# jdapena/distributed_point_functions

Measured on AMD Instinct MI355X. Metric: DPF leaf evals/sec, full-domain 2^30 uint64 at 1/2/4/8 GPUs; AES blocks/s, higher is better.
Workload: dtype u64

## Files before the change

distributed_point_functions_amd/csrc/kernels/dpf_device.h:

```cpp
#pragma once
#include <hip/hip_runtime.h>
#include <stdint.h>
#include <string.h>

#include "../../../include/dpf_hip.h"
#include "aes_core.h"

namespace {

struct T0Table {
  uint32_t v[256];
};
constexpr T0Table make_t0() {
  T0Table t{};
  for (int i = 0; i < 256; ++i) {
    uint32_t s = dpf_aes::kSbox[i];
    uint32_t s2 = ((s << 1) ^ ((s & 0x80) ? 0x1b : 0)) & 0xff;
    t.v[i] = s2 | (s << 8) | (s << 16) | ((s2 ^ s) << 24);
  }
  return t;
}
__constant__ T0Table c_t0 = make_t0();

struct RoundKeys {
// ... 136 lines not shown

struct ExpandParams {
  int64_t num_items;
  int num_levels;
  int k0;
  int S;
  const dpf_block* seeds_in;
  const uint8_t* ctrl_in;
  const dpf_block* cw_seed;
  const uint8_t* cw_left;
  const uint8_t* cw_right;
  char* out;
  RoundKeys rkl, rkr, rkv, rkd;
  int dyn_chunks;
  int ph_end[3];
  int64_t ph_item[3];
  unsigned int* chunk_counter;
  unsigned long long* clock;
};

__device__ __forceinline__ int64_t take_expand_chunk(const ExpandParams& p, int* lds_counter,
                                                     int64_t done, int& k0, int& S) {
  unsigned int c = 0;
  if ((threadIdx.x & 63) == 0)
    c = p.chunk_counter ? __hip_atomic_fetch_add(p.chunk_counter, 1u, __ATOMIC_RELAXED,
                                                 __HIP_MEMORY_SCOPE_AGENT)
                        : (unsigned int)atomicAdd(lds_counter, 1);
  c = __builtin_amdgcn_readfirstlane(c);
  const unsigned int e0 = (unsigned int)p.ph_end[0], e1 = (unsigned int)p.ph_end[1],
                     e2 = (unsigned int)p.ph_end[2];
  if (c >= e2) return done;
  const int j = (c >= e0) + (c >= e1);
  const unsigned int first = j == 0 ? 0u : (j == 1 ? e0 : e1);
  const unsigned int last = j == 0 ? e0 : (j == 1 ? e1 : e2);
  const int64_t item0 = j == 0 ? p.ph_item[0] : (j == 1 ? p.ph_item[1] : p.ph_item[2]);
  const int64_t group = p.chunk_counter ? 0 : (int64_t)blockIdx.x;
  const int64_t chunk = group * (int64_t)(last - first) + (c - first);
  k0 = p.k0 + 2 * j;
  S = p.S - 2 * j;
  return item0 + chunk * 64 + (int64_t)(threadIdx.x & 63);
}

__device__ __forceinline__ int64_t take_chunk(int* counter, int64_t per_wg, int64_t chunks,
                                              int64_t done) {
  int c = 0;
  if ((threadIdx.x & 63) == 0) c = atomicAdd(counter, 1);
  c = __builtin_amdgcn_readfirstlane(c);
  const int64_t g = (int64_t)blockIdx.x * per_wg + c;
  return c < per_wg && g < chunks ? g * 64 + (int64_t)(threadIdx.x & 63) : done;
}
// ... 901 lines not shown
```

distributed_point_functions_amd/csrc/kernels/dpf_expand_plan.hip:

```cpp
#include <stdint.h>

#include "../../../include/dpf_hip.h"
#include "dpf_runtime.h"

namespace dpf_rt {

int choose_subtree_depth(int64_t num_starts, int num_levels) {
  const int S = num_levels < max_subtree_depth() ? num_levels : max_subtree_depth();
#if defined(DPF_FORCE_S)
  if (num_levels >= DPF_FORCE_S) return DPF_FORCE_S;
#endif
  double best = -1;
  int best_s = S;
  for (int cand = S; cand >= (num_levels > 0 ? 1 : 0); --cand) {
    const int64_t items = num_starts << (num_levels - cand);
    const int blk = block_for(items);
    const int64_t threads = (int64_t)grid_for(items, blk) * blk;
    const int64_t rounds = (items + threads - 1) / threads;
    const double cost = (double)rounds * (2.0 * (num_levels - cand) + 3.0 * (double)(1ll << cand));
    if (best < 0 || cost < best * 0.999) {
      best = cost;
      best_s = cand;
    }
  }
// ... 2 lines not shown

bool small_shape(int64_t num_starts, int num_levels, int* t, int* D) {
  const int64_t cus = num_cus();
  if (hook_is("DPF_EXPAND_SMALL", '0') || num_levels < 1 || num_starts < 1 || num_starts > cus)
    return false;
  int tt = 0;
  while (tt < num_levels - 1 && (num_starts << (tt + 1)) <= cus) ++tt;
  const int d = num_levels - tt;
  if (d < 1 || d > kSmallMaxD) return false;
  *t = tt;
  *D = d;
  return true;
}

bool top_shape(int64_t num_items, int k0, int* t, int* D) {
  const int64_t starts = num_items >> k0;
  if (hook_is("DPF_EXPAND_TOP", '0') || k0 < 8 || starts > num_cus() ||
      num_items < 4 * (int64_t)num_cus())
    return false;
  int tt = 0;
  while ((starts << tt) < num_cus() && tt < k0 - 1) ++tt;
  if (k0 - tt > kSmallMaxD) tt = k0 - kSmallMaxD;
  if (k0 - tt < 1 || (starts << tt) > INT32_MAX) return false;
  *t = tt;
  *D = k0 - tt;
  return true;
}

static int octet_dynamic_shift(int S) {
  return hook_int("DPF_OCTET_DYNAMIC", S >= 11 ? 4 : 2, 0, 4);
}
int octet_walk_levels() { return hook_int("DPF_OCTET_WALK", 2, 0, 4); }
ChunkPlan plan_chunks(int64_t num_items, int k0, int S, int min_S, int64_t cus, bool sched_ok) {
  ChunkPlan c{};
  const int sh = octet_dynamic_shift(S);
  if (sh <= 0 || S - sh < min_S || k0 + sh > 62 || cus <= 0 || num_items <= 0 ||
      num_items > (INT64_MAX >> (sh + 4)) || (num_items << sh) % (cus * 64) != 0 ||
      (num_items << sh) < 4 * cus * max_block() || (num_items << sh) / 64 > (INT32_MAX >> 4))
    return c;
  c.shift = sh;
  const int big = sched_ok && (num_items << S) / cus >= ((int64_t)1 << 20);
  c.global = hook_int("DPF_OCTET_GLOBAL", big, 0, 1);
  c.groups = c.global ? 1 : cus;
  const int k = k0 + sh, s = S - sh;
  const int64_t coarse = (num_items << sh) / 64;
  const int finer = hook_int("DPF_OCTET_TAPER", big ? 2 : 0, 0, 2);
  const int64_t at = hook_int("DPF_OCTET_TAPER_AT", 2, 1, 16) * cus * (max_block() / 64);
  auto exists = [&](int j) { return j <= finer && s - 2 * j >= min_S && k + 2 * j <= 62; };
  int64_t start[4] = {0, coarse, coarse, coarse};
  if (exists(1)) start[1] = coarse - (coarse < at ? coarse : at);
  if (exists(2)) start[2] = coarse - (coarse - start[1] < (at >> 2) ? coarse - start[1] : (at >> 2));
  for (int j = 0; j < 3; ++j) {
    c.k0[j] = k + 2 * j;
    c.S[j] = s - 2 * j;
    c.chunks[j] = (start[j + 1] - start[j]) << (2 * j);
    c.first_item[j] = (start[j] * 64) << (2 * j);
  }
  return c;
}

void write_plan(const ChunkPlan& c, int64_t* out) {
  for (int i = 0; i < 15; ++i) out[i] = 0;
  out[0] = c.shift;
  if (!c.shift) return;
  out[1] = c.global;
  out[2] = c.groups;
  for (int j = 0; j < 3; ++j) {
    out[3 + 4 * j] = c.chunks[j];
    out[4 + 4 * j] = c.first_item[j];
    out[5 + 4 * j] = c.k0[j];
    out[6 + 4 * j] = c.S[j];
  }
}

}

using namespace dpf_rt;

extern "C" int dpf_hip_octet_schedule(int64_t num_items, int k0, int subtree_depth, int min_depth,
                                      int compute_units, int64_t* out) {
  if (!out) return fail(kInvalidArgument, "NULL pointer");
  if (num_items < 1 || k0 < 0 || subtree_depth < 0 || k0 + subtree_depth > 62 ||
      compute_units < 1)
    return fail(kInvalidArgument, "launch shape out of range");
  write_plan(plan_chunks(num_items, k0, subtree_depth, min_depth, compute_units, true), out);
  return kOk;
}
```

distributed_point_functions_amd/csrc/kernels/dpf_kernels.hip:

```cpp
#include <hip/hip_runtime.h>
#include <stdint.h>
#include <stdlib.h>
#include <string.h>

#include <atomic>
#include <type_traits>
#include <vector>
#include <string>

#include "../../../include/dpf_hip.h"
#include "dpf_device.h"
#include "dpf_dot.h"
#include "dpf_runtime.h"

namespace dpf_rt {
thread_local std::string g_last_error;
thread_local const char* g_last_expand = "";
thread_local int g_last_expand_s = -1;
thread_local int64_t g_last_dynamic_chunks = 0;
std::atomic<unsigned long long*> g_clock_acc{nullptr};

int fail(int code, const std::string& msg) {
  g_last_error = msg;
  return code;
// ... 58 lines not shown
      uint32_t bit = path_bit(path, p.num_levels - 1 - j);
      path_step(lk, lk.ks.l, lk.ks.d, s, t, bit, lds.cw_seed[j], lds.cw_ctrl[j]);
    }
    store_block(p.seeds_out + i, s);
    p.ctrl_out[i] = (uint8_t)t;
  }
}

template <class Leaf, bool SCHED = false>
__global__ __launch_bounds__(kBlock) DPF_WAVES_ATTR void expand_kernel(ExpandParams p, Leaf leaf) {
  __shared__ LdsImage lds;
  __shared__ int next_chunk;
  leaf.init();
  fill_tables(lds.tab);
  fill_cws(lds, p.cw_seed, p.cw_left, p.cw_right, p.num_levels);
  if (threadIdx.x == 0) next_chunk = 0;
  __syncthreads();
  const LdsLookup lk = make_lookup(lds, KeySet{key_ref(p.rkl), key_ref(p.rkr), key_ref(p.rkv), key_ref(p.rkd)});
  int k0 = p.k0, S = p.S;
  if constexpr (SCHED) ClockStamp::first_begin(p.clock);
  const int64_t nch = (p.num_items + 63) / 64;
  const int64_t end = SCHED ? INT64_MAX : p.num_items;
  auto take = [&]() -> int64_t {
    if constexpr (SCHED) return take_expand_chunk(p, &next_chunk, end, k0, S);
    else return take_chunk(&next_chunk, p.dyn_chunks, nch, p.num_items);
  };
  for (int64_t item = SCHED || p.dyn_chunks ? take()
                                            : blockIdx.x * (int64_t)blockDim.x + threadIdx.x;
       item < end;
       item = SCHED || p.dyn_chunks ? take() : item + (int64_t)gridDim.x * blockDim.x) {
    const int B = S >= 1 ? 1 : 0;
    const int G = S - B;
    const int64_t ngroups = (int64_t)1 << G;
    const int64_t r = item >> k0;
    Block4 s = load_block(p.seeds_in + r);
    uint32_t t = p.ctrl_in[r] & 1u;
    for (int j = 0; j < k0; ++j) {
      uint32_t bit = (uint32_t)((item >> (k0 - 1 - j)) & 1);
      path_step(lk, lk.ks.l, lk.ks.d, s, t, bit, lds.cw_seed[j], lds.cw_ctrl[j]);
    }
    Block4 sib[kGMax];
    uint32_t tb = 0;
    const int64_t leaf_base = item << S;
    for (int64_t g = 0; g < ngroups; ++g) {
      Block4 node = s;
      uint32_t nt = t;
      int ds = 0;
      if (g != 0) {
        ds = G - (int)__builtin_ctzll((unsigned long long)g);
#pragma unroll
        for (int d = 1; d <= kGMax; ++d)
          if (d == ds) { node = sib[d - 1]; nt = (tb >> d) & 1u; }
// ... 77 lines not shown
template <> struct OctetStash<SwarLeaf> { static constexpr int value = 1; };

template <class Leaf, bool SCHED = false>
__global__ __launch_bounds__(kBlock) DPF_WAVES_ATTR void expand_octet_kernel(ExpandParams p,
                                                                             Leaf leaf) {
  __shared__ LdsImage lds;
  constexpr int kStash = OctetStash<Leaf>::value;
  __shared__ uint4 stash[kBlock];
  __shared__ uint3 stash2[kStash >= 2 ? kBlock : 1];
  __shared__ int next_chunk;
  static_assert(sizeof(LdsImage) + 16 * kBlock + (kStash >= 2 ? 12 * kBlock : 0) + 16 <= 160 * 1024,
                "LDS over 160 KiB");
  leaf.init();
  fill_tables(lds.tab);
  fill_cws(lds, p.cw_seed, p.cw_left, p.cw_right, p.num_levels);
  if (threadIdx.x == 0) next_chunk = 0;
  __syncthreads();
  const LdsLookup lk = make_lookup(lds, KeySet{key_ref(p.rkl), key_ref(p.rkr), key_ref(p.rkv), key_ref(p.rkd)});
  int k0 = p.k0, S = p.S;
  ClockStamp stamp;
  stamp.begin(p.clock);
  const int lane = (int)(threadIdx.x & 63);
  const int64_t end = SCHED ? INT64_MAX : p.num_items;
  auto take = [&]() -> int64_t {
    if constexpr (SCHED) {
      return take_expand_chunk(p, &next_chunk, end, k0, S);
    } else {
      int c = 0;
      if (lane == 0) c = atomicAdd(&next_chunk, 1);
      c = __builtin_amdgcn_readfirstlane(c);
      return c < p.dyn_chunks ? ((int64_t)blockIdx.x * p.dyn_chunks + c) * 64 + lane
                              : p.num_items;
    }
  };
  for (int64_t item = SCHED || p.dyn_chunks ? take()
                                            : blockIdx.x * (int64_t)blockDim.x + threadIdx.x;
       item < end;
       item = SCHED || p.dyn_chunks ? take() : item + (int64_t)gridDim.x * blockDim.x) {
    const int G = S - 3;
    const int64_t ngroups = (int64_t)1 << G;
    const int64_t r = item >> k0;
    Block4 s = load_block(p.seeds_in + r);
    uint32_t t = p.ctrl_in[r] & 1u;
    for (int j = 0; j < k0; ++j) {
      const uint32_t bit = (uint32_t)((item >> (k0 - 1 - j)) & 1);
      path_step(lk, lk.ks.l, lk.ks.d, s, t, bit, lds.cw_seed[j], lds.cw_ctrl[j]);
    }
    Block4 sib[kGMax];
    uint32_t tb = 0;
    const int64_t leaf_base = item << S;
    Block4 next = s;
    for (int64_t g = 0; g < ngroups; ++g) {
      Block4 node = next;
      uint32_t nt = t;
      int ds = 0;
      if (g != 0) {
        ds = G - (int)__builtin_ctzll((unsigned long long)g);
        nt = (tb >> ds) & 1u;
      }
// ... 36 lines not shown
            q[2] = sib[kGMax - 2];
          }
          const uint4 v = stash[threadIdx.x];
          q[3] = Block4{v.x, v.y, v.z, v.w};
        }
        children_step_x2(lk, lk.ks.l, lk.ks.r, q[2 * hf], qt[2 * hf], q[2 * hf + 1],
                         qt[2 * hf + 1], lds.cw_seed[lvl + 2], lds.cw_ctrl[lvl + 2], l, lt);
        octet_half(leaf, lk, lk.ks.v, l, lt, leaf_base + 8 * g + 4 * hf, p.out, &sib[kGMax - 2]);
      }
    }
  }
  stamp.end(p.clock);
  if constexpr (HasFinish<Leaf>::value) leaf.finish();
}

template <class Leaf> struct IsFastInt : std::false_type {};
template <int BITS, bool XOR> struct IsFastInt<FastIntLeaf<BITS, XOR>> : std::true_type {};
template <int BITS, bool XOR> struct IsFastInt<DotLeaf<BITS, XOR>> : std::true_type {};
template <class Leaf>
__global__ __launch_bounds__(kBlock) DPF_WAVES_ATTR void expand_small_kernel(ExpandParams p, Leaf leaf) {
  __shared__ LdsImage lds;
  __shared__ uint4 nodes[kBlock];
  __shared__ uint32_t tbits[kBlock];
  leaf.init();
  fill_tables(lds.tab);
  fill_cws(lds, p.cw_seed, p.cw_left, p.cw_right, p.num_levels);
  __syncthreads();
  const LdsLookup lk =
      make_lookup(lds, KeySet{key_ref(p.rkl), key_ref(p.rkr), key_ref(p.rkv), key_ref(p.rkd)});
  const quad::Keys ql = quad::keys_of(p.rkl), qd = quad::keys_of(p.rkd);
// ... 63 lines not shown
      quad::children(lk, ql, qd, word(nodes[q], c), tbits[q], word(lds.cw_seed[lvl], c),
                     lds.cw_ctrl[lvl], c0, t0, c1, t1);
      quad::hash2(lk, qv, c0, c1);
      const Block4 h0 = quad::gather(c0), h1 = quad::gather(c1);
      if (c == 0) {
        leaf.store(leaf.correct(h0, t0), leaf0 + 2 * q, p.out);
        leaf.store(leaf.correct(h1, t1), leaf0 + 2 * q + 1, p.out);
      }
    }
  } else if (tid < npar) {
    const uint4 v = nodes[tid];
    Block4 c0, c1;
    uint32_t t0, t1;
    children_step(lk, lk.ks.l, lk.ks.r, Block4{v.x, v.y, v.z, v.w}, tbits[tid], lds.cw_seed[lvl],
                  lds.cw_ctrl[lvl], c0, t0, c1, t1);
    leaf.emit2(lk, lk.ks.v, c0, t0, c1, t1, leaf0 + 2 * tid, p.out);
  }
  if constexpr (HasFinish<Leaf>::value) leaf.finish();
}

struct SeedLeaf {
  dpf_block* seeds;
  uint8_t* ctrl;
  unsigned int* counter;
  __device__ __forceinline__ void init() const {
    if (counter != nullptr && blockIdx.x == 0 && threadIdx.x == 0) *counter = 0u;
  }
  __device__ __forceinline__ void emit2(const LdsLookup&, KeyRef, Block4 s0, uint32_t t0, Block4 s1,
                                        uint32_t t1, int64_t first, char*) const {
    store_block(seeds + first, s0);
    store_block(seeds + first + 1, s1);
    ctrl[first] = (uint8_t)t0;
    ctrl[first + 1] = (uint8_t)t1;
  }
};

__global__ void count_out_of_range_kernel(int64_t n, const dpf_block* __restrict__ pts, int log,
                                          unsigned long long* __restrict__ bad) {
  unsigned long long c = 0;
  for (int64_t i = blockIdx.x * (int64_t)blockDim.x + threadIdx.x; i < n;
       i += (int64_t)gridDim.x * blockDim.x) {
    const dpf_block b = pts[i];
    bool out;
    if (log >= 128) out = false;
    else if (log >= 64) out = (b.high >> (log - 64)) != 0;
    else out = b.high != 0 || (b.low >> log) != 0;
    c += out ? 1 : 0;
  }
// ... 140 lines not shown
  g_last_expand = name.c_str();
  g_last_expand_s = D;
  hipLaunchKernelGGL((expand_small_kernel<Leaf>), dim3((unsigned)p.num_items), dim3(kBlock), 0, s,
                     p, leaf);
  return true;
}


struct TopScratch {
  void* mem = nullptr;
  hipStream_t s = nullptr;
  ~TopScratch() {
    if (mem) (void)hipFreeAsync(mem, s);
  }
};
int expand_top(ExpandParams& p, hipStream_t s, TopScratch& scratch,
               unsigned int** counter = nullptr) {
  const int64_t starts = p.num_items >> p.k0;
  int t = 0, D = 0;
  if (!top_shape(p.num_items, p.k0, &t, &D)) return kOk;
  static const bool pool_kept = [] {
    int dev = 0;
    hipMemPool_t pool;
    if (hipGetDevice(&dev) != hipSuccess || hipDeviceGetDefaultMemPool(&pool, dev) != hipSuccess)
      return false;
    uint64_t keep = UINT64_MAX;
    return hipMemPoolSetAttribute(pool, hipMemPoolAttrReleaseThreshold, &keep) == hipSuccess;
  }();
  (void)pool_kept;
  const size_t items = (size_t)p.num_items;
  void* mem = nullptr;
  const size_t roots = (items * (sizeof(dpf_block) + 1) + 127) / 128 * 128;
  HIP_TRY(hipMallocAsync(&mem, roots + (counter ? 128 : 0), s));
  scratch.mem = mem;
  scratch.s = s;
  SeedLeaf leaf{static_cast<dpf_block*>(mem),
                static_cast<uint8_t*>(mem) + items * sizeof(dpf_block),
                counter ? reinterpret_cast<unsigned int*>(static_cast<char*>(mem) + roots)
                        : nullptr};
  if (counter) *counter = leaf.counter;
  ExpandParams q = p;
  q.k0 = t;
  q.S = D;
  q.num_levels = p.k0;
  q.num_items = starts << t;
  q.clock = nullptr;
  hipLaunchKernelGGL((expand_small_kernel<SeedLeaf>), dim3((unsigned)q.num_items), dim3(kBlock), 0,
                     s, q, leaf);
  HIP_TRY(hipGetLastError());
  p.seeds_in = leaf.seeds;
  p.ctrl_in = leaf.ctrl;
  p.cw_seed += p.k0;
  p.cw_left += p.k0;
  p.cw_right += p.k0;
  p.num_levels = p.S;
  p.k0 = 0;
  return kOk;
}

thread_local ChunkPlan g_last_plan{};
int subtree_shape(ExpandParams& p, int min_S, hipStream_t s, TopScratch& top, int* grid,
                  int* blk, bool sched_ok) {
  p.dyn_chunks = 0;
  p.chunk_counter = nullptr;
  g_last_plan = ChunkPlan{};
  const int64_t cus = num_cus();
  const ChunkPlan plan = plan_chunks(p.num_items, p.k0, p.S, min_S, cus, sched_ok);
  if (const int sh = plan.shift) {
    ExpandParams q = p;
    q.S -= sh;
    q.k0 += sh;
    q.num_items <<= sh;
    q.dyn_chunks = (int)(q.num_items / (cus * 64));
    int64_t taken = 0;
    for (int j = 0; j < 3; ++j) {
      taken += plan.chunks[j] / plan.groups;
      q.ph_end[j] = (int)taken;
      q.ph_item[j] = plan.first_item[j];
    }
    unsigned int* counter = nullptr;
    unsigned int** want_counter = plan.global ? &counter : nullptr;
    const int w = octet_walk_levels();
    int up = w > 0 && q.k0 - w >= 8 ? w : 0;
    ExpandParams t;
    for (;; up = 0) {
      t = q;
      t.k0 = q.k0 - up;
      t.S = q.S + up;
      t.num_items = q.num_items >> up;
      if (int st = expand_top(t, s, top, want_counter)) return st;
      if (t.k0 == 0 || up == 0) break;
    }
    if (t.k0 == 0) {
      q.chunk_counter = counter;
      q.seeds_in = t.seeds_in;
      q.ctrl_in = t.ctrl_in;
      q.cw_seed = t.cw_seed;
      q.cw_left = t.cw_left;
      q.cw_right = t.cw_right;
      q.num_levels = q.S + up;
      q.k0 = up;
      p = q;
      g_last_plan = plan;
      *grid = (int)cus;
      *blk = kBlock;
      return kOk;
    }
  }
  if (int st = expand_top(p, s, top)) return st;
  *blk = block_for(p.num_items);
  *grid = grid_for(p.num_items, *blk);
  return kOk;
}
template <class Leaf, bool OCTET> struct SchedDefault { static constexpr bool value = true; };
template <> struct SchedDefault<SwarLeaf, true> { static constexpr bool value = false; };
template <> struct SchedDefault<Mod32Leaf<kMod32MaxLeaves>, false> {
  static constexpr bool value = false;
};
bool has_schedule(const ExpandParams& p) {
  return p.dyn_chunks && (p.chunk_counter || p.ph_end[0] != p.ph_end[2]);
}
template <class Leaf> struct HasOctet : std::false_type {};
// ... 143 lines not shown
    sum += t;
    ++n;
  }
  out[0] = sec(~h[kProbeFirstExit]);
  out[1] = sec(h[kProbeLastExit]);
  out[2] = lo;
  out[3] = hi;
  out[4] = n ? sum / n : 0.0;
  out[5] = n;
  return kOk;
}

int dpf_hip_last_expand_schedule(int64_t* out) {
  if (!out) return fail(kInvalidArgument, "NULL pointer");
  dpf_rt::write_plan(g_last_plan, out);
  return kOk;
}

int dpf_hip_clock_probe_read(double* clock_ghz, int64_t* workgroups, double* mean_workgroup_s) {
  unsigned long long* acc = dpf_rt::g_clock_acc.load();
  if (!acc) return fail(kFailedPrecondition, "clock probe is off (dpf_hip_clock_probe(1))");
  unsigned long long h[4] = {0, 0, 0, 0};
  HIP_TRY(hipDeviceSynchronize());
  HIP_TRY(hipMemcpy(h, acc, sizeof(h), hipMemcpyDeviceToHost));
  HIP_TRY(hipMemset(acc, 0, kProbeBytes));
  HIP_TRY(hipDeviceSynchronize());
  if (clock_ghz) *clock_ghz = h[1] ? (double)h[0] / (double)h[1] * 0.1 : 0.0;
  if (workgroups) *workgroups = (int64_t)h[2];
  if (mean_workgroup_s) *mean_workgroup_s = h[2] ? (double)h[1] / (double)h[2] * 1e-8 : 0.0;
  return kOk;
// ... 238 lines not shown
```

distributed_point_functions_amd/csrc/kernels/dpf_runtime.h:

```cpp
#pragma once
#include <hip/hip_runtime.h>
#include <stdint.h>
#include <stdlib.h>

#include <string>
#include <type_traits>

#include "../../../include/dpf_hip.h"

namespace dpf_rt {

constexpr int kOk = 0, kInvalidArgument = 3, kResourceExhausted = 8, kFailedPrecondition = 9,
              kUnimplemented = 12, kInternal = 13;

int fail(int code, const std::string& msg);
int hip_fail(hipError_t e, const char* what);

inline bool hook_is(const char* name, char c) {
  const char* v = getenv(name);
  return v && v[0] == c;
}
inline bool hook_set(const char* name) { return getenv(name) != nullptr; }
inline long long hook_long(const char* name, long long dflt) {
  const char* v = getenv(name);
// ... 21 lines not shown
  switch (bits) {
    case 8: return f(std::integral_constant<int, 8>{});
    case 16: return f(std::integral_constant<int, 16>{});
    case 32: return f(std::integral_constant<int, 32>{});
    case 64: return f(std::integral_constant<int, 64>{});
    default: return f(std::integral_constant<int, 128>{});
  }
}
struct ChunkPlan {
  int shift;
  int global;
  int64_t groups;
  int k0[3], S[3];
  int64_t chunks[3], first_item[3];
};
ChunkPlan plan_chunks(int64_t num_items, int k0, int S, int min_S, int64_t cus, bool sched_ok);
void write_plan(const ChunkPlan& c, int64_t* out);
constexpr int kSmallMaxD = 11;
int choose_subtree_depth(int64_t num_starts, int num_levels);
bool small_shape(int64_t num_starts, int num_levels, int* t, int* D);
bool top_shape(int64_t num_items, int k0, int* t, int* D);
int octet_walk_levels();
int validate_desc(const dpf_value_desc* d);
int packed_size(const dpf_value_desc* d);
bool fast_int(const dpf_value_desc* d);

extern thread_local const char* g_last_dot;
int dot_type(const dpf_value_desc* d, int* words, int* xor_type);
int launch_dot_fold(int row_words, int xor_type, int accumulate, const void* workspace, void* out,
                    hipStream_t s);

constexpr int kHHSketchMaxRows = 2;
int launch_sketch_slot_weights(int64_t n, int64_t count, const int64_t* src_offset, int rows,
                               const uint32_t* weights, const uint32_t mod[2], uint32_t* out,
                               hipStream_t s);
int launch_hh_level(const dpf_prefix_batch_args& a, int b, hipStream_t s);
// ... 31 lines not shown
```

distributed_point_functions_amd/hip_abi.py:

```python
from __future__ import annotations

import ctypes
import os
import re
from typing import Optional, Sequence

import numpy as np

_HERE = os.path.dirname(os.path.abspath(__file__))
LIB_PATH = os.environ.get("DPF_HIP_LIB") or os.path.join(_HERE, "lib", "libdpf_hip.so")
HEADER = os.path.join(os.path.dirname(_HERE), "include", "dpf_hip.h")
MAX_LEAVES = 16
LEAF_INT, LEAF_INTMODN, LEAF_XOR = 0, 1, 2
MASK64 = (1 << 64) - 1

_lib = None


class DpfHipError(RuntimeError):
    def __init__(self, code: int, msg: str):
        super().__init__(f"[{code}] {msg}")
        self.code = code


# ... 73 lines not shown
        L.dpf_hip_sum_shares_u64.argtypes = [I64, I64, I, I, P, P, P]
        L.dpf_hip_packed_element_size.argtypes = [P]
        L.dpf_hip_event_create.argtypes = [ctypes.POINTER(ctypes.c_void_p)]
        L.dpf_hip_event_destroy.argtypes = [P]
        L.dpf_hip_event_record.argtypes = [P, P]
        L.dpf_hip_event_elapsed_ms.argtypes = [P, P, ctypes.POINTER(ctypes.c_float)]
        L.dpf_hip_stream_sync.argtypes = [P]
        L.dpf_hip_clock_probe.argtypes = [I]
        L.dpf_hip_clock_probe_read.argtypes = [ctypes.POINTER(ctypes.c_double),
                                               ctypes.POINTER(ctypes.c_int64),
                                               ctypes.POINTER(ctypes.c_double)]
        for name, types in (("dpf_hip_clock_probe_exits", [ctypes.POINTER(ctypes.c_double)]),
                            ("dpf_hip_octet_schedule",
                             [I64, I, I, I, I, ctypes.POINTER(ctypes.c_int64)]),
                            ("dpf_hip_last_expand_schedule", [ctypes.POINTER(ctypes.c_int64)]),
                            ("dpf_hip_last_dynamic_chunks", [ctypes.POINTER(ctypes.c_int64)]),
                            ("dpf_hip_mic_eval_batch",
                             [I64, I, P, P, P, P, P, I, P, P, I, P, I] + [P] * 11),
                            ("dpf_hip_expand_dot",
                             [I64, P, P, I, P, P, P, P, P, P, P, I, P, I, P, I, P, P, P]),
                            ("dpf_hip_dot_rows", [I64, I, P, P, P, I, P, P, P]),
                            ("dpf_hip_expand_dot_workspace_bytes", [P, I]),
                            ("dpf_hip_expand_dot_fused", [P, I]),
                            ("dpf_hip_last_dot_kernel", []),
                            ("dpf_hip_select_rows", [I64, I, I, P, I64, P, I, P, P, P]),
                            ("dpf_hip_select_workspace_bytes", [I, I]),
                            ("dpf_hip_last_select_shape", [ctypes.POINTER(ctypes.c_int64)]),
                            ("dpf_hip_dot_rows_batch", [I64, I, I, P, P, I64, P, I, P, P, P]),
                            ("dpf_hip_dot_rows_batch_workspace_bytes", [P, I, I]),
                            ("dpf_hip_last_dot_batch_shape", [ctypes.POINTER(ctypes.c_int64)]),
# ... 224 lines not shown

def octet_schedule(num_items: int, k0: int, subtree_depth: int, min_depth: int,
                   compute_units: int) -> dict:
    out = (ctypes.c_int64 * 15)()
    check(load().dpf_hip_octet_schedule(num_items, k0, subtree_depth, min_depth, compute_units,
                                        out))
    return _plan(out)


def last_expand_schedule() -> dict:
    out = (ctypes.c_int64 * 15)()
    check(load().dpf_hip_last_expand_schedule(out))
    return _plan(out)


def _plan(out) -> dict:
    phases = [{"chunks": out[3 + 4 * j], "first_item": out[4 + 4 * j], "k0": out[5 + 4 * j],
               "depth": out[6 + 4 * j]} for j in range(3) if out[3 + 4 * j]]
    return {"shift": out[0], "global": bool(out[1]), "counters": out[2], "phases": phases}


def check(st: int):
    if st != 0:
        raise DpfHipError(st, load().dpf_hip_last_error().decode())


def aes_key(k: int) -> AesKey:
    a = AesKey()
    for i, b in enumerate((k & ((1 << 128) - 1)).to_bytes(16, "little")):
        a.bytes[i] = b
# ... 286 lines not shown
```

include/dpf_hip.h:

```cpp
#ifndef DPF_HIP_H_
#define DPF_HIP_H_

#include <stddef.h>
#include <stdint.h>

#ifdef __cplusplus
extern "C" {
#endif

#define DPF_HIP_ABI_VERSION 2
#define DPF_MAX_LEAVES 16

typedef struct dpf_block {
  uint64_t low;
  uint64_t high;
} dpf_block;

typedef struct dpf_aes_key {
  uint8_t bytes[16];
} dpf_aes_key;

enum dpf_leaf_kind { DPF_LEAF_INT = 0, DPF_LEAF_INTMODN = 1, DPF_LEAF_XOR = 2 };

typedef struct dpf_value_desc {
// ... 86 lines not shown
int dpf_hip_dot_rows_batch_workspace_bytes(const dpf_value_desc* desc, int record_words,
                                           int num_queries);
int dpf_hip_last_dot_batch_shape(int64_t* out3);

const char* dpf_hip_last_expand_kernel(int* subtree_depth);

int dpf_hip_clock_probe(int on);
int dpf_hip_clock_probe_read(double* clock_ghz, int64_t* workgroups, double* mean_workgroup_s);

int dpf_hip_clock_probe_exits(double* out);

int dpf_hip_octet_schedule(int64_t num_items, int k0, int subtree_depth, int min_depth,
                           int compute_units, int64_t* out);

int dpf_hip_last_expand_schedule(int64_t* out);

const char* dpf_hip_last_batch_kernel(void);

const char* dpf_hip_last_points_kernel(void);

int dpf_hip_last_dynamic_chunks(int64_t* per_wg);

int dpf_hip_eval_points(int64_t num_points, int64_t points_per_key, int num_levels,
                        const dpf_block* key_seed, const uint8_t* party,
                        const dpf_block* seeds_in, const uint8_t* control_in,
                        const dpf_block* tree_index, const int32_t* block_index,
                        const dpf_block* cw_seed, const uint8_t* cw_left,
                        const uint8_t* cw_right, const dpf_aes_key* key_left,
                        const dpf_aes_key* key_right, const dpf_aes_key* key_value,
                        const dpf_value_desc* desc, const dpf_block* value_correction,
// ... 216 lines not shown
```

Before: 72.56 billion.

## Precompute per-phase root seeds in top pass so tapered chunks skip path walk

The top expansion pass now writes root seeds laid out per taper phase, expanding extra tail levels for the finer phases. Expand kernels then start from a phase-specific root and walk only the remaining levels instead of recomputing the path from the coarse root. The first chunk per wave is assigned statically, without an atomic, and tapering is enabled for medium-sized shapes too. This trades a larger root scratch buffer and more top-pass AES work for less redundant path walking and fewer counter atomics, at the cost of added planning complexity.

```diff
diff --git a/distributed_point_functions_amd/csrc/kernels/dpf_device.h b/distributed_point_functions_amd/csrc/kernels/dpf_device.h
--- a/distributed_point_functions_amd/csrc/kernels/dpf_device.h
+++ b/distributed_point_functions_amd/csrc/kernels/dpf_device.h
@@ -174,18 +174,25 @@
   RoundKeys rkl, rkr, rkv, rkd;
   int dyn_chunks;
   int ph_end[3];
+  int ph_walk[3];
   int64_t ph_item[3];
+  int64_t ph_root[3];
   unsigned int* chunk_counter;
   unsigned long long* clock;
 };
 
 __device__ __forceinline__ int64_t take_expand_chunk(const ExpandParams& p, int* lds_counter,
-                                                     int64_t done, int& k0, int& S) {
+                                                     bool first_take, int64_t done, int& k0,
+                                                     int& S, int& walk, int64_t& root) {
   unsigned int c = 0;
-  if ((threadIdx.x & 63) == 0)
+  if (first_take) {
+    const unsigned int w = threadIdx.x >> 6;
+    c = p.chunk_counter ? blockIdx.x * (blockDim.x >> 6) + w : w;
+  } else if ((threadIdx.x & 63) == 0) {
     c = p.chunk_counter ? __hip_atomic_fetch_add(p.chunk_counter, 1u, __ATOMIC_RELAXED,
                                                  __HIP_MEMORY_SCOPE_AGENT)
                         : (unsigned int)atomicAdd(lds_counter, 1);
+  }
   c = __builtin_amdgcn_readfirstlane(c);
   const unsigned int e0 = (unsigned int)p.ph_end[0], e1 = (unsigned int)p.ph_end[1],
                      e2 = (unsigned int)p.ph_end[2];
@@ -194,6 +201,8 @@
   const unsigned int first = j == 0 ? 0u : (j == 1 ? e0 : e1);
   const unsigned int last = j == 0 ? e0 : (j == 1 ? e1 : e2);
   const int64_t item0 = j == 0 ? p.ph_item[0] : (j == 1 ? p.ph_item[1] : p.ph_item[2]);
+  root = j == 0 ? p.ph_root[0] : (j == 1 ? p.ph_root[1] : p.ph_root[2]);
+  walk = j == 0 ? p.ph_walk[0] : (j == 1 ? p.ph_walk[1] : p.ph_walk[2]);
   const int64_t group = p.chunk_counter ? 0 : (int64_t)blockIdx.x;
   const int64_t chunk = group * (int64_t)(last - first) + (c - first);
   k0 = p.k0 + 2 * j;
diff --git a/distributed_point_functions_amd/csrc/kernels/dpf_expand_plan.hip b/distributed_point_functions_amd/csrc/kernels/dpf_expand_plan.hip
--- a/distributed_point_functions_amd/csrc/kernels/dpf_expand_plan.hip
+++ b/distributed_point_functions_amd/csrc/kernels/dpf_expand_plan.hip
@@ -40,12 +40,14 @@
 }
 
 bool top_shape(int64_t num_items, int k0, int* t, int* D) {
+  return top_shape_for(num_items, k0, num_cus(), t, D);
+}
+bool top_shape_for(int64_t num_items, int k0, int64_t cus, int* t, int* D) {
   const int64_t starts = num_items >> k0;
-  if (hook_is("DPF_EXPAND_TOP", '0') || k0 < 8 || starts > num_cus() ||
-      num_items < 4 * (int64_t)num_cus())
+  if (hook_is("DPF_EXPAND_TOP", '0') || k0 < 8 || starts > cus || num_items < 4 * cus)
     return false;
   int tt = 0;
-  while ((starts << tt) < num_cus() && tt < k0 - 1) ++tt;
+  while ((starts << tt) < cus && tt < k0 - 1) ++tt;
   if (k0 - tt > kSmallMaxD) tt = k0 - kSmallMaxD;
   if (k0 - tt < 1 || (starts << tt) > INT32_MAX) return false;
   *t = tt;
@@ -57,7 +59,8 @@
   return hook_int("DPF_OCTET_DYNAMIC", S >= 11 ? 4 : 2, 0, 4);
 }
 int octet_walk_levels() { return hook_int("DPF_OCTET_WALK", 2, 0, 4); }
-ChunkPlan plan_chunks(int64_t num_items, int k0, int S, int min_S, int64_t cus, bool sched_ok) {
+ChunkPlan plan_chunks(int64_t num_items, int k0, int S, int min_S, int64_t cus, bool sched_ok,
+                      bool phase_roots) {
   ChunkPlan c{};
   const int sh = octet_dynamic_shift(S);
   if (sh <= 0 || S - sh < min_S || k0 + sh > 62 || cus <= 0 || num_items <= 0 ||
@@ -70,8 +73,11 @@
   c.groups = c.global ? 1 : cus;
   const int k = k0 + sh, s = S - sh;
   const int64_t coarse = (num_items << sh) / 64;
-  const int finer = hook_int("DPF_OCTET_TAPER", big ? 2 : 0, 0, 2);
-  const int64_t at = hook_int("DPF_OCTET_TAPER_AT", 2, 1, 16) * cus * (max_block() / 64);
+  const int small_taper =
+      phase_roots && sched_ok && !big && (num_items << S) / cus >= ((int64_t)1 << 19);
+  const int finer = hook_int("DPF_OCTET_TAPER", big || small_taper ? 2 : 0, 0, 2);
+  const int64_t at =
+      hook_int("DPF_OCTET_TAPER_AT", small_taper ? 1 : 2, 1, 16) * cus * (max_block() / 64);
   auto exists = [&](int j) { return j <= finer && s - 2 * j >= min_S && k + 2 * j <= 62; };
   int64_t start[4] = {0, coarse, coarse, coarse};
   if (exists(1)) start[1] = coarse - (coarse < at ? coarse : at);
@@ -99,9 +105,103 @@
   }
 }
 
+static bool plan_roots(ChunkPlan& c, int up, int64_t cus, RootPlan* r) {
+  const int k = c.k0[0];
+  if (up < 0 || up > k) return false;
+  const int64_t coarse = (c.first_item[2] >> 4) / 64 + c.chunks[2] / 16;
+  int t = 0, D = 0;
+  if (!top_shape_for((coarse * 64) >> up, k - up, cus, &t, &D)) return false;
+  int64_t unit = D + up > 6 ? (int64_t)1 << (D + up - 6) : 1;
+  if (!c.global) {
+    int64_t a = unit, b = cus;
+    while (b) { const int64_t m = a % b; a = b; b = m; }
+    unit = unit / a * cus;
+  }
+  int64_t start[4] = {0, (c.first_item[1] >> 2) / 64, (c.first_item[2] >> 4) / 64, coarse};
+  for (int j = 1; j < 3; ++j)
+    if (start[j] < coarse) start[j] -= start[j] % unit;
+  const int max_tail = hook_int("DPF_OCTET_TAIL", 2, 0, 4);
+  RootPlan o{};
+  o.up = up;
+  o.t = t;
+  o.D = D;
+  o.wgs = ((coarse * 64) >> up) >> D;
+  o.waves = cus * (max_block() / 64);
+  for (int j = 0; j < 3; ++j) {
+    c.chunks[j] = (start[j + 1] - start[j]) << (2 * j);
+    c.first_item[j] = (start[j] * 64) << (2 * j);
+    o.tail[j] = 2 * j < max_tail ? 2 * j : max_tail;
+    o.walk[j] = up + 2 * j - o.tail[j];
+    o.depth[j] = c.k0[j] - o.walk[j];
+    o.first_root[j] = c.first_item[j] >> o.walk[j];
+    o.roots[j] = (c.chunks[j] * 64) >> o.walk[j];
+    o.base[j] = o.total;
+    o.total += o.roots[j];
+  }
+  int64_t next = o.wgs;
+  for (int j = 2; j >= 0; --j) {
+    if (o.roots[j]) next = (o.first_root[j] >> o.tail[j]) >> D;
+    o.first_wg[j] = next;
+  }
+  *r = o;
+  return true;
+}
+
+bool plan_launch(int64_t num_items, int k0, int S, int min_S, int64_t cus, bool sched_ok,
+                 ChunkPlan* c, RootPlan* r) {
+  const ChunkPlan plan = plan_chunks(num_items, k0, S, min_S, cus, sched_ok, true);
+  if (!plan.shift) return false;
+  const int w = octet_walk_levels();
+  for (int up = w > 0 && plan.k0[0] - w >= 8 ? w : 0;; up = 0) {
+    *c = plan;
+    if (plan_roots(*c, up, cus, r)) return true;
+    if (up == 0) return false;
+  }
+}
+
+void write_roots(const ChunkPlan& c, const RootPlan& r, int64_t* out) {
+  for (int i = 0; i < kRootPlanWords; ++i) out[i] = 0;
+  if (!c.shift) return;
+  out[0] = 1;
+  out[1] = r.up;
+  out[2] = r.t;
+  out[3] = r.D;
+  out[4] = r.wgs;
+  out[5] = r.total;
+  out[6] = r.waves;
+  out[7] = c.global;
+  for (int j = 0; j < 3; ++j) {
+    int64_t* o = out + 8 + 10 * j;
+    o[0] = c.chunks[j];
+    o[1] = c.first_item[j];
+    o[2] = r.depth[j];
+    o[3] = r.first_root[j];
+    o[4] = r.roots[j];
+    o[5] = r.base[j];
+    o[6] = r.tail[j];
+    o[7] = r.first_wg[j];
+    o[8] = r.walk[j];
+    o[9] = c.S[j];
+  }
+}
+
 }
 
 using namespace dpf_rt;
+
+extern "C" int dpf_hip_octet_roots(int64_t num_items, int k0, int subtree_depth, int min_depth,
+                                   int compute_units, int64_t* out) {
+  if (!out) return fail(kInvalidArgument, "NULL pointer");
+  if (num_items < 1 || k0 < 0 || subtree_depth < 0 || k0 + subtree_depth > 62 ||
+      compute_units < 1)
+    return fail(kInvalidArgument, "launch shape out of range");
+  ChunkPlan c{};
+  RootPlan r{};
+  if (!plan_launch(num_items, k0, subtree_depth, min_depth, compute_units, true, &c, &r))
+    c = ChunkPlan{};
+  write_roots(c, r, out);
+  return kOk;
+}
 
 extern "C" int dpf_hip_octet_schedule(int64_t num_items, int k0, int subtree_depth, int min_depth,
                                       int compute_units, int64_t* out) {
@@ -109,6 +209,6 @@
   if (num_items < 1 || k0 < 0 || subtree_depth < 0 || k0 + subtree_depth > 62 ||
       compute_units < 1)
     return fail(kInvalidArgument, "launch shape out of range");
-  write_plan(plan_chunks(num_items, k0, subtree_depth, min_depth, compute_units, true), out);
+  write_plan(plan_chunks(num_items, k0, subtree_depth, min_depth, compute_units, true, false), out);
   return kOk;
 }
diff --git a/distributed_point_functions_amd/csrc/kernels/dpf_kernels.hip b/distributed_point_functions_amd/csrc/kernels/dpf_kernels.hip
--- a/distributed_point_functions_amd/csrc/kernels/dpf_kernels.hip
+++ b/distributed_point_functions_amd/csrc/kernels/dpf_kernels.hip
@@ -96,28 +96,30 @@
   leaf.init();
   fill_tables(lds.tab);
   fill_cws(lds, p.cw_seed, p.cw_left, p.cw_right, p.num_levels);
-  if (threadIdx.x == 0) next_chunk = 0;
+  if (threadIdx.x == 0) next_chunk = SCHED ? (int)(blockDim.x >> 6) : 0;
   __syncthreads();
   const LdsLookup lk = make_lookup(lds, KeySet{key_ref(p.rkl), key_ref(p.rkr), key_ref(p.rkv), key_ref(p.rkd)});
   int k0 = p.k0, S = p.S;
+  int64_t root = 0;
+  int walk = p.k0;
   if constexpr (SCHED) ClockStamp::first_begin(p.clock);
   const int64_t nch = (p.num_items + 63) / 64;
   const int64_t end = SCHED ? INT64_MAX : p.num_items;
-  auto take = [&]() -> int64_t {
-    if constexpr (SCHED) return take_expand_chunk(p, &next_chunk, end, k0, S);
+  auto take = [&](bool first_take) -> int64_t {
+    if constexpr (SCHED) return take_expand_chunk(p, &next_chunk, first_take, end, k0, S, walk, root);
     else return take_chunk(&next_chunk, p.dyn_chunks, nch, p.num_items);
   };
-  for (int64_t item = SCHED || p.dyn_chunks ? take()
+  for (int64_t item = SCHED || p.dyn_chunks ? take(true)
                                             : blockIdx.x * (int64_t)blockDim.x + threadIdx.x;
        item < end;
-       item = SCHED || p.dyn_chunks ? take() : item + (int64_t)gridDim.x * blockDim.x) {
+       item = SCHED || p.dyn_chunks ? take(false) : item + (int64_t)gridDim.x * blockDim.x) {
     const int B = S >= 1 ? 1 : 0;
     const int G = S - B;
     const int64_t ngroups = (int64_t)1 << G;
-    const int64_t r = item >> k0;
+    const int64_t r = SCHED ? root + (item >> walk) : item >> k0;
     Block4 s = load_block(p.seeds_in + r);
     uint32_t t = p.ctrl_in[r] & 1u;
-    for (int j = 0; j < k0; ++j) {
+    for (int j = SCHED ? k0 - walk : 0; j < k0; ++j) {
       uint32_t bit = (uint32_t)((item >> (k0 - 1 - j)) & 1);
       path_step(lk, lk.ks.l, lk.ks.d, s, t, bit, lds.cw_seed[j], lds.cw_ctrl[j]);
     }
@@ -225,17 +227,19 @@
   leaf.init();
   fill_tables(lds.tab);
   fill_cws(lds, p.cw_seed, p.cw_left, p.cw_right, p.num_levels);
-  if (threadIdx.x == 0) next_chunk = 0;
+  if (threadIdx.x == 0) next_chunk = SCHED ? (int)(blockDim.x >> 6) : 0;
   __syncthreads();
   const LdsLookup lk = make_lookup(lds, KeySet{key_ref(p.rkl), key_ref(p.rkr), key_ref(p.rkv), key_ref(p.rkd)});
   int k0 = p.k0, S = p.S;
+  int64_t root = 0;
+  int walk = p.k0;
   ClockStamp stamp;
   stamp.begin(p.clock);
   const int lane = (int)(threadIdx.x & 63);
   const int64_t end = SCHED ? INT64_MAX : p.num_items;
-  auto take = [&]() -> int64_t {
+  auto take = [&](bool first_take) -> int64_t {
     if constexpr (SCHED) {
-      return take_expand_chunk(p, &next_chunk, end, k0, S);
+      return take_expand_chunk(p, &next_chunk, first_take, end, k0, S, walk, root);
     } else {
       int c = 0;
       if (lane == 0) c = atomicAdd(&next_chunk, 1);
@@ -244,16 +248,16 @@
                               : p.num_items;
     }
   };
-  for (int64_t item = SCHED || p.dyn_chunks ? take()
+  for (int64_t item = SCHED || p.dyn_chunks ? take(true)
                                             : blockIdx.x * (int64_t)blockDim.x + threadIdx.x;
        item < end;
-       item = SCHED || p.dyn_chunks ? take() : item + (int64_t)gridDim.x * blockDim.x) {
+       item = SCHED || p.dyn_chunks ? take(false) : item + (int64_t)gridDim.x * blockDim.x) {
     const int G = S - 3;
     const int64_t ngroups = (int64_t)1 << G;
-    const int64_t r = item >> k0;
+    const int64_t r = SCHED ? root + (item >> walk) : item >> k0;
     Block4 s = load_block(p.seeds_in + r);
     uint32_t t = p.ctrl_in[r] & 1u;
-    for (int j = 0; j < k0; ++j) {
+    for (int j = SCHED ? k0 - walk : 0; j < k0; ++j) {
       const uint32_t bit = (uint32_t)((item >> (k0 - 1 - j)) & 1);
       path_step(lk, lk.ks.l, lk.ks.d, s, t, bit, lds.cw_seed[j], lds.cw_ctrl[j]);
     }
@@ -320,6 +324,7 @@
   if constexpr (HasFinish<Leaf>::value) leaf.finish();
 }
 
+struct SeedLeaf;
 template <class Leaf> struct IsFastInt : std::false_type {};
 template <int BITS, bool XOR> struct IsFastInt<FastIntLeaf<BITS, XOR>> : std::true_type {};
 template <int BITS, bool XOR> struct IsFastInt<DotLeaf<BITS, XOR>> : std::true_type {};
@@ -413,7 +418,10 @@
     uint32_t t0, t1;
     children_step(lk, lk.ks.l, lk.ks.r, Block4{v.x, v.y, v.z, v.w}, tbits[tid], lds.cw_seed[lvl],
                   lds.cw_ctrl[lvl], c0, t0, c1, t1);
-    leaf.emit2(lk, lk.ks.v, c0, t0, c1, t1, leaf0 + 2 * tid, p.out);
+    if constexpr (std::is_same_v<Leaf, SeedLeaf>)
+      leaf.roots(lk, lds, lvl + 1, c0, t0, c1, t1, leaf0 + 2 * tid);
+    else
+      leaf.emit2(lk, lk.ks.v, c0, t0, c1, t1, leaf0 + 2 * tid, p.out);
   }
   if constexpr (HasFinish<Leaf>::value) leaf.finish();
 }
@@ -422,15 +430,68 @@
   dpf_block* seeds;
   uint8_t* ctrl;
   unsigned int* counter;
+  unsigned int counter_first;
+  unsigned int ph_wg[2];
+  int ph_tail[3];
+  int64_t ph_root[3];
   __device__ __forceinline__ void init() const {
-    if (counter != nullptr && blockIdx.x == 0 && threadIdx.x == 0) *counter = 0u;
-  }
-  __device__ __forceinline__ void emit2(const LdsLookup&, KeyRef, Block4 s0, uint32_t t0, Block4 s1,
-                                        uint32_t t1, int64_t first, char*) const {
-    store_block(seeds + first, s0);
-    store_block(seeds + first + 1, s1);
-    ctrl[first] = (uint8_t)t0;
-    ctrl[first + 1] = (uint8_t)t1;
+    if (counter != nullptr && blockIdx.x == 0 && threadIdx.x == 0) *counter = counter_first;
+  }
+  __device__ __forceinline__ void put(int64_t slot, Block4 s, uint32_t t) const {
+    store_block(seeds + slot, s);
+    ctrl[slot] = (uint8_t)t;
+  }
+  __device__ __forceinline__ void roots(const LdsLookup& lk, const LdsImage& lds, int lvl, Block4 a,
+                                        uint32_t ta, Block4 b, uint32_t tb, int64_t first) const {
+    const int j = (blockIdx.x >= ph_wg[0]) + (blockIdx.x >= ph_wg[1]);
+    const int64_t off = j == 0 ? ph_root[0] : (j == 1 ? ph_root[1] : ph_root[2]);
+    if (j == 0) {
+      put(off + first, a, ta);
+      put(off + first + 1, b, tb);
+      return;
+    }
+    const int e = j == 1 ? ph_tail[1] : ph_tail[2], G = e - 1;
+    if (e == 0) {
+      put(off + first, a, ta);
+      put(off + first + 1, b, tb);
+      return;
+    }
+    const int64_t slot_a = off + (first << e), slot_b = slot_a + ((int64_t)1 << e);
+    constexpr int kTailG = 3;
+    Block4 sa[kTailG], sb[kTailG];
+    uint32_t bits_a = 0, bits_b = 0;
+    for (int g = 0; g < (1 << G); ++g) {
+      Block4 na = a, nb = b;
+      uint32_t nta = ta, ntb = tb;
+      int ds = 0;
+      if (g != 0) {
+        ds = G - __builtin_ctz((unsigned)g);
+#pragma unroll
+        for (int d = 1; d <= kTailG; ++d)
+          if (d == ds) { na = sa[d - 1]; nb = sb[d - 1]; }
+        nta = (bits_a >> ds) & 1u;
+        ntb = (bits_b >> ds) & 1u;
+      }
+      Block4 c[4];
+      uint32_t ct[4];
+      for (int d = ds; d < G; ++d) {
+        children_step_x2(lk, lk.ks.l, lk.ks.r, na, nta, nb, ntb, lds.cw_seed[lvl + d],
+                         lds.cw_ctrl[lvl + d], c, ct);
+#pragma unroll
+        for (int x = 1; x <= kTailG; ++x)
+          if (x == d + 1) { sa[x - 1] = c[1]; sb[x - 1] = c[3]; }
+        bits_a = (bits_a & ~(1u << (d + 1))) | (ct[1] << (d + 1));
+        bits_b = (bits_b & ~(1u << (d + 1))) | (ct[3] << (d + 1));
+        na = c[0]; nta = ct[0];
+        nb = c[2]; ntb = ct[2];
+      }
+      children_step_x2(lk, lk.ks.l, lk.ks.r, na, nta, nb, ntb, lds.cw_seed[lvl + G],
+                       lds.cw_ctrl[lvl + G], c, ct);
+      put(slot_a + 2 * g, c[0], ct[0]);
+      put(slot_a + 2 * g + 1, c[1], ct[1]);
+      put(slot_b + 2 * g, c[2], ct[2]);
+      put(slot_b + 2 * g + 1, c[3], ct[3]);
+    }
   }
 };
 
@@ -601,11 +662,16 @@
     if (mem) (void)hipFreeAsync(mem, s);
   }
 };
-int expand_top(ExpandParams& p, hipStream_t s, TopScratch& scratch,
+int expand_top(ExpandParams& p, hipStream_t s, TopScratch& scratch, const RootPlan* rp = nullptr,
                unsigned int** counter = nullptr) {
   const int64_t starts = p.num_items >> p.k0;
   int t = 0, D = 0;
-  if (!top_shape(p.num_items, p.k0, &t, &D)) return kOk;
+  if (rp) {
+    t = rp->t;
+    D = rp->D;
+  } else if (!top_shape(p.num_items, p.k0, &t, &D)) {
+    return kOk;
+  }
   static const bool pool_kept = [] {
     int dev = 0;
     hipMemPool_t pool;
@@ -615,21 +681,33 @@
     return hipMemPoolSetAttribute(pool, hipMemPoolAttrReleaseThreshold, &keep) == hipSuccess;
   }();
   (void)pool_kept;
-  const size_t items = (size_t)p.num_items;
+  const size_t items = (size_t)(rp ? rp->total : p.num_items);
   void* mem = nullptr;
   const size_t roots = (items * (sizeof(dpf_block) + 1) + 127) / 128 * 128;
   HIP_TRY(hipMallocAsync(&mem, roots + (counter ? 128 : 0), s));
   scratch.mem = mem;
   scratch.s = s;
-  SeedLeaf leaf{static_cast<dpf_block*>(mem),
-                static_cast<uint8_t*>(mem) + items * sizeof(dpf_block),
-                counter ? reinterpret_cast<unsigned int*>(static_cast<char*>(mem) + roots)
-                        : nullptr};
+  SeedLeaf leaf{};
+  leaf.seeds = static_cast<dpf_block*>(mem);
+  leaf.ctrl = static_cast<uint8_t*>(mem) + items * sizeof(dpf_block);
+  leaf.counter =
+      counter ? reinterpret_cast<unsigned int*>(static_cast<char*>(mem) + roots) : nullptr;
+  leaf.ph_wg[0] = leaf.ph_wg[1] = UINT32_MAX;
+  int tail = 0;
+  if (rp) {
+    leaf.counter_first = (unsigned int)rp->waves;
+    for (int j = 0; j < 3; ++j) {
+      leaf.ph_root[j] = rp->base[j] - rp->first_root[j];
+      leaf.ph_tail[j] = rp->tail[j];
+      if (j > 0) leaf.ph_wg[j - 1] = (unsigned int)rp->first_wg[j];
+      if (rp->roots[j] && rp->tail[j] > tail) tail = rp->tail[j];
+    }
+  }
   if (counter) *counter = leaf.counter;
   ExpandParams q = p;
   q.k0 = t;
   q.S = D;
-  q.num_levels = p.k0;
+  q.num_levels = p.k0 + tail;
   q.num_items = starts << t;
   q.clock = nullptr;
   hipLaunchKernelGGL((expand_small_kernel<SeedLeaf>), dim3((unsigned)q.num_items), dim3(kBlock), 0,
@@ -646,14 +724,18 @@
 }
 
 thread_local ChunkPlan g_last_plan{};
+thread_local RootPlan g_last_roots{};
 int subtree_shape(ExpandParams& p, int min_S, hipStream_t s, TopScratch& top, int* grid,
                   int* blk, bool sched_ok) {
   p.dyn_chunks = 0;
   p.chunk_counter = nullptr;
   g_last_plan = ChunkPlan{};
+  g_last_roots = RootPlan{};
   const int64_t cus = num_cus();
-  const ChunkPlan plan = plan_chunks(p.num_items, p.k0, p.S, min_S, cus, sched_ok);
-  if (const int sh = plan.shift) {
+  ChunkPlan plan{};
+  RootPlan rp{};
+  if (plan_launch(p.num_items, p.k0, p.S, min_S, cus, sched_ok, &plan, &rp)) {
+    const int sh = plan.shift, up = rp.up;
     ExpandParams q = p;
     q.S -= sh;
     q.k0 += sh;
@@ -664,35 +746,29 @@
       taken += plan.chunks[j] / plan.groups;
       q.ph_end[j] = (int)taken;
       q.ph_item[j] = plan.first_item[j];
-    }
+      q.ph_root[j] = rp.base[j] - rp.first_root[j];
+      q.ph_walk[j] = rp.walk[j];
+    }
+    ExpandParams t = q;
+    t.k0 = q.k0 - up;
+    t.S = q.S + up;
+    t.num_items = q.num_items >> up;
     unsigned int* counter = nullptr;
-    unsigned int** want_counter = plan.global ? &counter : nullptr;
-    const int w = octet_walk_levels();
-    int up = w > 0 && q.k0 - w >= 8 ? w : 0;
-    ExpandParams t;
-    for (;; up = 0) {
-      t = q;
-      t.k0 = q.k0 - up;
-      t.S = q.S + up;
-      t.num_items = q.num_items >> up;
-      if (int st = expand_top(t, s, top, want_counter)) return st;
-      if (t.k0 == 0 || up == 0) break;
-    }
-    if (t.k0 == 0) {
-      q.chunk_counter = counter;
-      q.seeds_in = t.seeds_in;
-      q.ctrl_in = t.ctrl_in;
-      q.cw_seed = t.cw_seed;
-      q.cw_left = t.cw_left;
-      q.cw_right = t.cw_right;
-      q.num_levels = q.S + up;
-      q.k0 = up;
-      p = q;
-      g_last_plan = plan;
-      *grid = (int)cus;
-      *blk = kBlock;
-      return kOk;
-    }
+    if (int st = expand_top(t, s, top, &rp, plan.global ? &counter : nullptr)) return st;
+    q.chunk_counter = counter;
+    q.seeds_in = t.seeds_in;
+    q.ctrl_in = t.ctrl_in;
+    q.cw_seed = t.cw_seed;
+    q.cw_left = t.cw_left;
+    q.cw_right = t.cw_right;
+    q.num_levels = q.S + up;
+    q.k0 = up;
+    p = q;
+    g_last_plan = plan;
+    g_last_roots = rp;
+    *grid = (int)cus;
+    *blk = kBlock;
+    return kOk;
   }
   if (int st = expand_top(p, s, top)) return st;
   *blk = block_for(p.num_items);
@@ -866,6 +942,12 @@
 int dpf_hip_last_expand_schedule(int64_t* out) {
   if (!out) return fail(kInvalidArgument, "NULL pointer");
   dpf_rt::write_plan(g_last_plan, out);
+  return kOk;
+}
+
+int dpf_hip_last_expand_roots(int64_t* out) {
+  if (!out) return fail(kInvalidArgument, "NULL pointer");
+  dpf_rt::write_roots(g_last_plan, g_last_roots, out);
   return kOk;
 }
 
diff --git a/distributed_point_functions_amd/csrc/kernels/dpf_runtime.h b/distributed_point_functions_amd/csrc/kernels/dpf_runtime.h
--- a/distributed_point_functions_amd/csrc/kernels/dpf_runtime.h
+++ b/distributed_point_functions_amd/csrc/kernels/dpf_runtime.h
@@ -59,12 +59,24 @@
   int k0[3], S[3];
   int64_t chunks[3], first_item[3];
 };
-ChunkPlan plan_chunks(int64_t num_items, int k0, int S, int min_S, int64_t cus, bool sched_ok);
+ChunkPlan plan_chunks(int64_t num_items, int k0, int S, int min_S, int64_t cus, bool sched_ok,
+                      bool phase_roots);
 void write_plan(const ChunkPlan& c, int64_t* out);
+struct RootPlan {
+  int up, t, D;
+  int tail[3], walk[3], depth[3];
+  int64_t wgs, total, waves;
+  int64_t first_root[3], roots[3], base[3], first_wg[3];
+};
+bool plan_launch(int64_t num_items, int k0, int S, int min_S, int64_t cus, bool sched_ok,
+                 ChunkPlan* c, RootPlan* r);
+constexpr int kRootPlanWords = 38;
+void write_roots(const ChunkPlan& c, const RootPlan& r, int64_t* out);
 constexpr int kSmallMaxD = 11;
 int choose_subtree_depth(int64_t num_starts, int num_levels);
 bool small_shape(int64_t num_starts, int num_levels, int* t, int* D);
 bool top_shape(int64_t num_items, int k0, int* t, int* D);
+bool top_shape_for(int64_t num_items, int k0, int64_t cus, int* t, int* D);
 int octet_walk_levels();
 int validate_desc(const dpf_value_desc* d);
 int packed_size(const dpf_value_desc* d);
diff --git a/distributed_point_functions_amd/hip_abi.py b/distributed_point_functions_amd/hip_abi.py
--- a/distributed_point_functions_amd/hip_abi.py
+++ b/distributed_point_functions_amd/hip_abi.py
@@ -111,6 +111,9 @@
                             ("dpf_hip_octet_schedule",
                              [I64, I, I, I, I, ctypes.POINTER(ctypes.c_int64)]),
                             ("dpf_hip_last_expand_schedule", [ctypes.POINTER(ctypes.c_int64)]),
+                            ("dpf_hip_octet_roots",
+                             [I64, I, I, I, I, ctypes.POINTER(ctypes.c_int64)]),
+                            ("dpf_hip_last_expand_roots", [ctypes.POINTER(ctypes.c_int64)]),
                             ("dpf_hip_last_dynamic_chunks", [ctypes.POINTER(ctypes.c_int64)]),
                             ("dpf_hip_mic_eval_batch",
                              [I64, I, P, P, P, P, P, I, P, P, I, P, I] + [P] * 11),
@@ -365,6 +368,28 @@
     return _plan(out)
 
 
+def octet_roots(num_items: int, k0: int, subtree_depth: int, min_depth: int,
+                compute_units: int) -> dict:
+    out = (ctypes.c_int64 * 38)()
+    check(load().dpf_hip_octet_roots(num_items, k0, subtree_depth, min_depth, compute_units, out))
+    return _roots(out)
+
+
+def last_expand_roots() -> dict:
+    out = (ctypes.c_int64 * 38)()
+    check(load().dpf_hip_last_expand_roots(out))
+    return _roots(out)
+
+
+def _roots(out) -> dict:
+    names = ("chunks", "first_item", "root_depth", "first_root", "roots", "slot", "tail",
+             "first_workgroup", "walk", "depth")
+    phases = [dict(zip(names, out[8 + 10 * j:18 + 10 * j])) for j in range(3) if out[8 + 10 * j]]
+    return {"dynamic": bool(out[0]), "walk": out[1], "pass_t": out[2], "pass_lds_levels": out[3],
+            "pass_workgroups": out[4], "roots": out[5], "waves": out[6], "global": bool(out[7]),
+            "phases": phases}
+
+
 def _plan(out) -> dict:
     phases = [{"chunks": out[3 + 4 * j], "first_item": out[4 + 4 * j], "k0": out[5 + 4 * j],
                "depth": out[6 + 4 * j]} for j in range(3) if out[3 + 4 * j]]
diff --git a/include/dpf_hip.h b/include/dpf_hip.h
--- a/include/dpf_hip.h
+++ b/include/dpf_hip.h
@@ -124,6 +124,10 @@
                            int compute_units, int64_t* out);
 
 int dpf_hip_last_expand_schedule(int64_t* out);
+
+int dpf_hip_octet_roots(int64_t num_items, int k0, int subtree_depth, int min_depth,
+                        int compute_units, int64_t* out);
+int dpf_hip_last_expand_roots(int64_t* out);
 
 const char* dpf_hip_last_batch_kernel(void);
 
```

Result: no change. 73.03 billion, median of 6 (+0.6%).
